# EmreAdabag/osqp

Measured on AMD Instinct MI355X. Metric: ADMM iters/sec (single QP), higher is better.
Workload: dtype f64; 1 GPU; config2 random sparse QP n=10000 m=20000 nnzA=200000 nnzPtriu=59985, one step = osqp_update_rho(0.1) + cold-started osqp_solve; adaptive_rho_interval=100, status=solved, graph_launches=4775, resident_gave_up=0, resident_slow_waits=0, parallelism=replicas x1 (a single QP does not shard)

## Files before the change

include/osqp_amd_engine.h:

```cpp
#ifndef OSQP_AMD_ENGINE_H
#define OSQP_AMD_ENGINE_H

#include "osqp_amd_types.h"

#ifdef __cplusplus
extern "C" {
#endif

#define HIPENG_OK            0
#define HIPENG_ERR_NO_DEVICE (-101)
#define HIPENG_ERR_HIP       (-102)
#define HIPENG_ERR_ARG       (-103)
#define HIPENG_ERR_ALLOC     (-104)

typedef struct hipeng hipeng;

typedef struct {
  c_float sigma;
  c_float alpha;
  c_float pcg_eps_rel;
  c_float pcg_eps_abs;
  c_int   pcg_max_iter;
  c_int   no_restart;
} hipeng_params;
// ... 14 lines not shown
} hipeng_scalars;

typedef struct {
  c_int admm_done;
  c_int pcg_iters_total;
  c_int pcg_iters_last;
  c_int pcg_iters_max;
  c_int pcg_forced;
  c_int graph_launches;
  c_int kernels_per_pcg_iter;
  c_int neg_curvature;
  c_int resident;
} hipeng_stats;

int hipeng_create(hipeng **out, const csc *P, const csc *A, const c_float *q,
                  const c_float *l, const c_float *u, const c_float *rho_vec,
                  const hipeng_params *prm, int device);
void hipeng_destroy(hipeng *e);

int hipeng_set_params(hipeng *e, const hipeng_params *prm);
int hipeng_set_scaling(hipeng *e, const c_float *D, const c_float *E, c_float c);
int hipeng_ruiz_scale(hipeng *e, c_int passes, c_float *D, c_float *E, c_float *cost,
                      c_float *q, c_float *l, c_float *u, c_float *Px, c_float *Ax);
int hipeng_matrices_changed(hipeng *e);
int hipeng_upload_q(hipeng *e, const c_float *q);
int hipeng_upload_bounds(hipeng *e, const c_float *l, const c_float *u);
int hipeng_upload_rho(hipeng *e, const c_float *rho_vec);
int hipeng_upload_matrices(hipeng *e, const csc *P, const csc *A);
int hipeng_cold_start(hipeng *e);
int hipeng_set_iterates(hipeng *e, const c_float *x, const c_float *y);
int hipeng_set_z(hipeng *e, const c_float *z);

int hipeng_run_admm(hipeng *e, c_int count);
int hipeng_residuals(hipeng *e, hipeng_scalars *out);
int hipeng_certificates(hipeng *e, c_float eps_dx, int unscaled, hipeng_scalars *inout);
int hipeng_download(hipeng *e, c_float *x, c_float *y, c_float *z, c_float *dx,
                    c_float *dy, int dy_projected);
int hipeng_get_stats(hipeng *e, hipeng_stats *st);
int hipeng_reset_stats(hipeng *e);
int hipeng_sync(hipeng *e);

int hipeng_kkt_solve(hipeng *e, c_float *b);
int hipeng_kkt_solve_unrefined(hipeng *e, c_float *b);

int hipeng_spmv(hipeng *e, int which, const c_float *x, c_float *y);
int hipeng_spmv_dev(hipeng *e, int which, const c_float *d_x, c_float *d_y);
int hipeng_time_kernel(hipeng *e, int which, int reps, double *usec);
int hipeng_kernel_bytes(hipeng *e, int which, double *bytes);
int hipeng_is_split(hipeng *e);
int hipeng_pcg_layout(hipeng *e, long long out[16]);
int hipeng_row_eliminated(hipeng *e, c_int i);
c_int hipeng_elim_count(hipeng *e);
int hipeng_resident_info(hipeng *e, long long out[16]);
int hipeng_resident_plan(const csc *P, const csc *A, int nwg, long long stats[8], int *Kptr, int *Kcol, int *kdst, long long cap,
                         unsigned short *rowpos, unsigned short *slotcol, int *wg4);
long long hipeng_resident_dump(hipeng *e, int *row, int *col, double *val, long long cap);

int hipeng_dense_invert_selftest(int n, const double *A, double *Ainv, double *ms);

typedef struct hipsens hipsens;
int hipsens_create(hipsens **out, c_int n, c_int m, c_int nnzP, c_int nnzA, int device);
void hipsens_destroy(hipsens *s);
int hipsens_set_point(hipsens *s, hipeng *pe, const c_float *x, const c_float *yact, const c_int *act,
                      const c_float *D, const c_float *E, c_float c);
int hipsens_grad(hipsens *s, hipeng *pe, const csc *P, const csc *A, const c_float *rx, const c_float *rnu,
                 c_float *dPx, c_float *dAx);
int hipsens_tan_rhs(hipsens *s, hipeng *pe, const csc *P, const csc *A, c_int ndir, const c_float *dq, const c_float *dl,
                    const c_float *du, const c_float *dPx, const c_float *dAx, c_float *g);

#ifdef __cplusplus
}
#endif
#endif
```

osqp_amd/csrc/engine.hip:

```cpp
#include <hip/hip_runtime.h>
#include <cstdio>
#include <new>
#include <cstdlib>
#include <cstring>
#include <cmath>
#include <vector>
#include <map>
#include <algorithm>
#include <mutex>
#include <condition_variable>
#include <thread>
#include <atomic>
#include <chrono>
#include "../../include/osqp_amd_engine.h"

#define TB 256
#define MAX_CHUNK 2048
#define LONG_ROW 512
#define HUGE_ROW 8192
#define MAX_PARTS 1024
#define MAX_HUGE_FOLD 4
#define INF_BOUND 1e26

#define HIPCHK(call)                                                            \
// ... 9 lines not shown
struct RowBlk { int r0, r1, k0, k1; };
#define IS_LONG(b) ((b).r1 - (b).r0 == 1 && (b).k1 - (b).k0 >= LONG_ROW)
struct __attribute__((aligned(32))) G4 { double r, w, s, m; };

struct DevMat {
  int nrows, nblk;
  int nstream;
  int nwave;
  const int    *rowptr;
  const int    *col;
  const unsigned short *col16;
  const double *val;
  const int    *split;
  const RowBlk *blk;
};

#define DENSE_MAX 128
struct DenseBlk { int c0, b, off, pitch; };
struct DenseP {
  int nblk;
  const DenseBlk *blk;
  const double *val;
};

struct State {
  int    run;
  int    done;
  int    stalled;
  int    neg_curv;
  int    iters[2];
  int    neg_curv_seen;
  int    iters_last;
  int    iters_max;
  int    iters_min;
  int    forced;
  long long iters_total;
  long long admm_done;
  double rz[2];
  double tol2;
  double gam[2], alp[2];
  int    hist_r;
  long long admm_target;
  unsigned res_epoch;
  int    res_fail;
  int    res_pipe_off;
  int    res_chk_fail;
  int    res_dbg[4];
  int    res_slow;
  int    res_slow_max;
  int    res_repub;
  int    res_slow_hist[4];
  unsigned res_slow_xcc;
  int    res_slow_last[4];
};

struct Params {
  double sigma, alpha, eps_rel, eps_abs, cinv;
  int    pcg_max_iter, use_cvec, has_scaling, pad0;
  double ex_theta;
  int    ex_h0, ex_h1;
  int    no_restart;
};

struct Ctx {
  int n, m;
  DevMat A, M;
  DevMat Mk;
  DenseP dP;
  int nh, hrow[MAX_HUGE_FOLD];
  const double *hcol;
  int gridA, gridM;
  double *xy, *z, *zt, *va, *vb, *q, *l, *u, *rho, *rhoinv, *minv, *pdiag;
  double *r, *zz, *kp, *pt0, *pt1, *dxy, *dy, *cvec;
  double *init_r, *init_z;
  double *vx, *vold;
  double *pdir, *ut;
  G4     *g4;
  int     init_stride;
  int     fin_wave_rows;
  double *vd;
  int     plain_rhs;
  const int *plain_skip;
  const unsigned short *u0map;
  double *u0pos;
  int     nelim;
  const int *erow, *ecol, *epos;
  double *rhoe, *ecoef, *edinv, *xte;
  double *D, *Dinv, *E, *Einv;
  double *part_rz, *part_rr, *part_bb, *part_pkp, *part_s0, *part_s1, *part_s2, *part_gam, *part_del;
  const double *fin_rr;
  int fin_cnt;
  double *scal;
  double *part_h;
  State  *st;
  const Params *prm;
#ifdef OSQP_AMD_TIMELINE
  unsigned long long *tl;
#endif
};

#ifdef OSQP_AMD_TIMELINE
#define TL_CAP (1 << 20)
#define TL_MARK(c, id) do { if (blockIdx.x == 0 && threadIdx.x == 0) { const unsigned long long k_ = atomicAdd((c).tl, 1ull); \
    if (k_ < TL_CAP - 2) (c).tl[1 + k_] = ((unsigned long long)(id) << 56) | (wall_clock64() & 0x00FFFFFFFFFFFFFFull); } } while (0)
#define TLK_N 10
#define TLK_DECL long long tlk_[TLK_N], tll_[2] = {0, 0}; for (int q_ = 0; q_ < TLK_N; ++q_) tlk_[q_] = 0
// ... 860 lines not shown
    TLK_AT(7, 0);
    for (int i = i0 + TB / RL; i < b.r1; i += TB / RL) {
      const double zt = row_sum_par(lprod, c.A.rowptr[i] - b.k0, c.A.rowptr[i + 1] - b.k0, rlane, RL);
      if (rlane == 0) row_update(i, zt);
    }
    __syncthreads();
  }
  for (int bi = blockIdx.x + gridDim.x; bi < c.A.nstream; bi += gridDim.x) {
    const RowBlk bb = c.A.blk[bi];
    stage_products<1>(c.A, bb, xts, nullptr, lprod, nullptr);
    __syncthreads();
    const int RLb = lanes_for(bb.r1 - bb.r0), rgb = threadIdx.x / RLb, rlb = threadIdx.x % RLb;
    for (int i = bb.r0 + rgb; i < bb.r1; i += TB / RLb) {
      const double zt = row_sum_par(lprod, c.A.rowptr[i] - bb.k0, c.A.rowptr[i + 1] - bb.k0, rlb, RLb);
      if (rlb == 0) row_update(i, zt);
    }
    __syncthreads();
  }
  if (c.fin_wave_rows) {
    const int lane = threadIdx.x & 63, wv = threadIdx.x >> 6;
    for (int bi = c.A.nstream + blockIdx.x * (TB / 64) + wv; bi < c.A.nwave; bi += gridDim.x * (TB / 64)) {
      const RowBlk lb = c.A.blk[bi];
      const double zt = wave_row_dot(c.A, lb.k0, lb.k1, [&](int cc) { return xts[cc]; });
      if (lane == 0) row_update(lb.r0, zt);
    }
  } else
  for (int bi = c.A.nstream + blockIdx.x; bi < c.A.nwave; bi += gridDim.x) {
    const RowBlk lb = c.A.blk[bi];
    const double zt = long_row_dot(c.A, lb.k0, lb.k1, xts, red);
    if (threadIdx.x == 0) row_update(lb.r0, zt);
    __syncthreads();
  }
  for (int bi = c.A.nwave + blockIdx.x; bi < c.A.nblk; bi += gridDim.x) {
    const double zt = huge_row_sum(c, bi, red);
    if (threadIdx.x == 0) row_update(c.A.blk[bi].r0, zt);
    __syncthreads();
  }
  TLK_AT(8, 0); TLK_LAST(1);
  TLK_FLUSH(c, 110, 9);
}


#define RES_TB 512
#define RES_PT (RES_TB - 64)
#define RES_MAXROWS 61
#define RES_MAXN (RES_MAXROWS * 256)
#define RES_MAXPAD 16384
#define RES_MAXLD (RES_MAXPAD / 2 / RES_TB)
#define RES_WAIT_TICKS 2000000LL
#define RES_SLOW_TICKS 5000LL
#define AUX_SC1 16
#define AUX_VOL ((int)0x80000000)
#define RES_DBG 16
#define RES_FSTRIDE 32
#define RES_GSTRIDE 16
typedef unsigned int u32x4 __attribute__((ext_vector_type(4)));
typedef unsigned int u32x2 __attribute__((ext_vector_type(2)));
struct ResWG { int r0, nr, cnt, pos; };
struct ResCtx {
  int nwg, E, npad;
  int npw;
  const unsigned short *rowpos;
  int pipe;
  int u0_direct;
  int inject;
  const ResWG *wg;
  double *val;
  const unsigned short *col;
  const unsigned char *rowl;
  const int *krp, *kcj, *kps, *kdst;
  const unsigned long long *brk;
  const unsigned short *slot0;
  const unsigned short *segrow;
  double *ubuf;
  unsigned *flags;
  int *dbg;
  double *sbuf;
};

static __device__ __forceinline__ __amdgpu_buffer_rsrc_t res_rsrc(const void *p, size_t bytes) {
  return __builtin_amdgcn_make_buffer_rsrc(const_cast<void *>(p), 0, (int)bytes, 0x00020000);
}

__device__ __forceinline__ int res_spin_check(State *st, long long &t0, int &late) {
  const long long now = wall_clock64();
  const long long el = now - t0;
  if (el < 0 || el > (1LL << 40)) { t0 = now; late = 0; return 0; }
  if (__hip_atomic_load(&st->res_fail, __ATOMIC_RELAXED, __HIP_MEMORY_SCOPE_AGENT)) return 2;
  if (el > RES_WAIT_TICKS) { if (late) return 1; late = 1; } else late = 0;
  return 0;
}
__device__ __forceinline__ void res_note(State *st, int *dbg, int g, int verdict, int kind, int nx, int first, unsigned seen, long long t0, unsigned rounds, int gidx) {
  if (verdict == 1 && atomicCAS(&st->res_dbg[0], 0, kind) == 0) { st->res_dbg[1] = nx; st->res_dbg[2] = g; st->res_dbg[3] = first; }
  int *d = dbg + (size_t)RES_DBG * g;
  const long long now = wall_clock64();
  d[3] = verdict == 1 ? kind : 3; d[4] = first; d[5] = (int)seen; d[6] = (int)(now - t0);
  d[7] = (int)__builtin_amdgcn_s_getreg((3 << 11) | 20);
  d[8] = (int)(unsigned)now; d[9] = (int)rounds; d[10] = gidx;
}
__device__ __forceinline__ void res_slow_note(State *st, long long t0, int nx, int g, int missed, int kind) {
  const long long el = wall_clock64() - t0;
  if (el > RES_SLOW_TICKS && el < (1LL << 40)) {
    atomicAdd(&st->res_slow, 1); atomicMax(&st->res_slow_max, (int)(el > 0x7fffffffLL ? 0x7fffffffLL : el));
    atomicAdd(&st->res_slow_hist[el < 20000 ? 0 : (el < 50000 ? 1 : (el < 200000 ? 2 : 3))], 1);
    atomicOr(&st->res_slow_xcc, 1u << (__builtin_amdgcn_s_getreg((3 << 11) | 20) & 15));
    st->res_slow_last[0] = nx; st->res_slow_last[1] = g; st->res_slow_last[2] = missed; st->res_slow_last[3] = kind;
  }
}

__device__ __forceinline__ int lane_int(int v, int l) { return __builtin_amdgcn_readlane(v, l); }
__global__ void __launch_bounds__(TB) k_form_K(Ctx c, ResCtx rc) {
  const double sigma = c.prm->sigma;
  if (blockIdx.x == 0 && threadIdx.x == 0) c.st->res_pipe_off = 0;
  const int lane = threadIdx.x & 63, nwaves = gridDim.x * (TB / 64);
  for (int i = blockIdx.x * (TB / 64) + (threadIdx.x >> 6); i < c.n; i += nwaves) {
    const int e0 = rc.krp[i], e1 = rc.krp[i + 1];
    const int ka = c.M.split[i], kb = c.M.rowptr[i + 1];
    for (int eb = e0; eb < e1; eb += 256) {
      int j[4]; double v[4];
#pragma unroll
      for (int q = 0; q < 4; ++q) {
        const int idx = eb + q * 64 + lane;
        j[q] = -1; v[q] = 0.0;
        if (idx < e1) {
          j[q] = rc.kcj[idx];
          const int ps = rc.kps[idx];
          v[q] = (ps >= 0 ? c.M.val[ps] : 0.0) + (j[q] == i ? sigma : 0.0);
        }
      }
      for (int kc = ka; kc < kb; kc += 64) {
        const bool on = kc + lane < kb;
        const int kk = on ? c.M.col[kc + lane] - c.n : 0;
        const double ai = on ? c.M.val[kc + lane] : 0.0, rk = on ? c.rhoe[kk] : 0.0;
        const int p0 = on ? c.A.rowptr[kk] : 0, p1 = on ? c.A.rowptr[kk + 1] : 0;
        const int cnt = min(64, kb - kc);
        for (int q = 0; q < cnt; ++q) {
          const double a_i = lane_value(ai, q), r = lane_value(rk, q);
          const int s0 = lane_int(p0, q), s1 = lane_int(p1, q);
          for (int ec = s0; ec < s1; ec += 64) {
            const bool eon = ec + lane < s1;
            const int cj = eon ? c.A.col[ec + lane] : -1;
            const double av = eon ? c.A.val[ec + lane] : 0.0;
            const int len = min(64, s1 - ec);
            for (int e = 0; e < len; ++e) {
              const int cjb = lane_int(cj, e);
              const double t = r * (a_i * lane_value(av, e));
#pragma unroll
              for (int q4 = 0; q4 < 4; ++q4) if (j[q4] == cjb) v[q4] += t;
            }
          }
        }
      }
      const bool igone = c.nelim && c.erow[i] >= 0;
#pragma unroll
      for (int q = 0; q < 4; ++q) {
        const int idx = eb + q * 64 + lane;
        if (idx < e1) {
          const bool gone = c.nelim && (igone || c.erow[j[q]] >= 0);
          rc.val[rc.kdst[idx]] = gone ? (j[q] == i ? 1.0 : 0.0) : v[q];
        }
      }
    }
  }
}

template <int E>
__global__ void __launch_bounds__(RES_TB) k_pcg_resident(Ctx c, ResCtx rc) {
  extern __shared__ __attribute__((aligned(16))) double rlds[];
  State *st = c.st;
  TL_MARK(c, 5);
  if (st->stalled || !st->run || st->res_fail) return;
  double *uv = rlds;
  double *seg = uv + rc.npad;
  double *sc = seg + RES_TB + RES_MAXROWS;
  double *sval = sc + 8;
#ifdef OSQP_AMD_TIMELINE
  long long *tls = reinterpret_cast<long long *>(sval + 768);
#define RTL(k) do { if (blockIdx.x == 0 && threadIdx.x == 0 && nx >= 1 && nx <= 64) tls[(nx - 1) * 5 + (k)] = wall_clock64(); } while (0)
  long long *wtl = tls + 5 * 64;
#define WTL(k) do { if (blockIdx.x == 0 && (threadIdx.x & 63) == 0 && (nx == 8 || nx == 1)) wtl[(nx == 1 ? 40 : 0) + (k) * 8 + (threadIdx.x >> 6)] = wall_clock64(); } while (0)
  if (blockIdx.x == 0 && threadIdx.x == 0) wtl[80] = wall_clock64();
#else
#define RTL(k) do { } while (0)
#define WTL(k) do { } while (0)
#endif
  const int g = blockIdx.x, t = threadIdx.x, lane = t & 63, wv = t >> 6;
  const int nwg = rc.nwg, npad = rc.npad;
  const ResWG w = rc.wg[g];
  const Params prm = *c.prm;
  const unsigned ep0 = st->res_epoch;
  const bool sabotage = rc.inject > 0 && g == rc.nwg - 1 && st->admm_done + 1 == rc.inject;
  bool pipe = rc.pipe && !st->res_pipe_off && !prm.no_restart;
  const bool prod = wv != 0;
  const int tt = t - 64;
  double kv[E]; unsigned short kc[E];
#pragma unroll
  for (int k = 0; k < E; ++k) { kv[k] = 0.0; kc[k] = 0; }
  unsigned long long brk = 0ull;
  int slot0 = 0;
  if (prod) {
#pragma unroll
    for (int k = 0; k < E; ++k) {
      const size_t idx = ((size_t)g * E + k) * RES_PT + tt;
      kv[k] = rc.val[idx]; kc[k] = rc.col[idx];
    }
    brk = rc.brk[(size_t)g * RES_PT + tt];
    slot0 = rc.slot0[(size_t)g * RES_PT + tt];
  }
  int sr0 = 0, sr1 = 0;
  int ppos[4];
#pragma unroll
  for (int q = 0; q < 4; ++q) { const int o = lane + 64 * q; ppos[q] = 0; if (o < rc.nwg) { const ResWG wo = rc.wg[o]; ppos[q] = wo.pos + wo.nr; } }
  double rr0 = 0.0, bb = 0.0;
  for (int i = lane; i < c.gridM; i += 64) { rr0 += c.part_rr[i]; bb += c.part_bb[i]; }
  rr0 = wave_sum(rr0); bb = wave_sum(bb);
  const double tol2 = fmax(prm.eps_rel * prm.eps_rel * bb, prm.eps_abs * prm.eps_abs);
  if (rr0 <= tol2) {
    if (g == 0 && t == 0) { st->done = 1; st->tol2 = tol2; }
    return;
  }
  const bool own = wv == 0 && lane < w.nr;
  const int j = w.r0 + lane;
  double r_ = 0, u_ = 0, w_ = 0, p_ = 0, s_ = 0, x_ = 0, mi = 0, x0_ = 0, r0_ = 0;
  double z_ = 0, q_ = 0;
  if (own) {
    r_ = c.init_r[(size_t)j * c.init_stride]; u_ = c.init_z[j]; x_ = c.vx[j]; mi = c.minv[j];
    x0_ = x_; r0_ = r_;
    sr0 = rc.segrow[(size_t)g * (RES_MAXROWS + 1) + lane]; sr1 = rc.segrow[(size_t)g * (RES_MAXROWS + 1) + lane + 1];
  }
  if (t == 0) sc[3] = 0.0;
  __syncthreads();
  int nx = 0;
  unsigned tag = ep0;
  int par = 0;

  auto vec_exchange = [&](double val, bool ride) __attribute__((always_inline)) -> bool {
    double e0 = 0.0, e1 = 0.0, e2 = 0.0;
    ++nx; tag = ep0 + (unsigned)nx; par = (int)(tag & 1u);
    if (sabotage && nx == 3) return false;
    RTL(0);
    const __amdgpu_buffer_rsrc_t rs = res_rsrc(rc.ubuf + (size_t)par * npad, (size_t)npad * 8);
    if (wv == 0) {
      if (lane < w.nr) {
        u32x2 d; d.x = (unsigned)__double2loint(val); d.y = (unsigned)__double2hiint(val);
        __builtin_amdgcn_raw_buffer_store_b64(d, rs, (w.pos + lane) * 8, 0, AUX_SC1);
      }
      if (ride) { e0 = wave_sum(own ? r_ * u_ : 0.0); e1 = wave_sum(own ? w_ * u_ : 0.0); e2 = wave_sum(own ? r_ * r_ : 0.0); }
      if (lane < 3) {
        const double v = lane == 0 ? e0 : (lane == 1 ? e1 : e2);
        u32x2 d; d.x = (unsigned)__double2loint(v); d.y = (unsigned)__double2hiint(v);
        __builtin_amdgcn_raw_buffer_store_b64(d, rs, (w.pos + w.nr + lane) * 8, 0, AUX_SC1);
      }
      asm volatile("s_waitcnt vmcnt(0)" ::: "memory");
      if (lane == 0) __hip_atomic_store(rc.flags + (size_t)g * RES_FSTRIDE, tag, __ATOMIC_RELAXED, __HIP_MEMORY_SCOPE_AGENT);
    }
    if (wv < rc.npw) {
      const int o = t;
      bool pend = o < nwg && o != g;
      int miss16 = -1;
      unsigned seen = 0, rounds = 0;
      long long t0 = wall_clock64();
      int late = 0;
      bool gave = false;
      while (true) {
        if (pend) {
          seen = __hip_atomic_load(rc.flags + (size_t)o * RES_FSTRIDE, __ATOMIC_RELAXED, __HIP_MEMORY_SCOPE_AGENT);
          pend = (int)(seen - tag) < 0;
        }
        if (!__any(pend)) break;
        if (++rounds & 15u) { __builtin_amdgcn_s_sleep(1); continue; }
        const int verdict = res_spin_check(st, t0, late);
        if (verdict) {
          const unsigned long long miss = __ballot(pend);
          const int fl = miss ? (int)__ffsll((long long)miss) - 1 : 0;
          const unsigned sv = (unsigned)__builtin_amdgcn_readlane((int)seen, fl);
          if (lane == 0) { res_note(st, rc.dbg, g, verdict, 1, nx, miss ? 64 * wv + fl : -1, sv, t0, rounds, 0); sc[3] = 1.0; }
          gave = true;
// ... 95 lines not shown
      int late = 0;
      bool gave = false;
      while (true) {
        u32x2 gv[6];
#pragma unroll
        for (int q = 0; q < 6; ++q) if (pend & (1u << q)) gv[q] = __builtin_amdgcn_raw_buffer_load_b64(rg, (o * RES_GSTRIDE + q) * 8, 0, AUX_SC1 | AUX_VOL);
#pragma unroll
        for (int q = 0; q < 6; ++q)
          if (pend & (1u << q)) { if (gv[q].y == tag) { svw[q] = gv[q].x; pend &= ~(1u << q); } else seen = gv[q].y; }
        if (!__any(pend != 0)) break;
        asm volatile("" ::: "memory");
        if (++rounds & 15u) { __builtin_amdgcn_s_sleep(1); continue; }
        const int verdict = res_spin_check(st, t0, late);
        if (verdict) {
          const unsigned long long miss = __ballot(pend != 0);
          const int fl = miss ? (int)__ffsll((long long)miss) - 1 : 0;
          const unsigned sv = (unsigned)__builtin_amdgcn_readlane((int)seen, fl);
          const int gi = __builtin_amdgcn_readlane((int)pend, fl);
          if (lane == 0) { res_note(st, rc.dbg, g, verdict, 2, nx, miss ? 64 * wv + fl : -1, sv, t0, rounds, gi); sc[3] = 1.0; }
          gave = true;
          break;
        }
        if (rounds == 16u) { const unsigned long long ms = __ballot(pend != 0); miss16 = ms ? 64 * wv + (int)__ffsll((long long)ms) - 1 : -1; }
        if ((rounds & 63u) == 0 && wv == 0) {
          if (lane < 6) {
            const double v = lane < 2 ? pg : (lane < 4 ? pd : prr);
            const unsigned half = (lane & 1) ? (unsigned)__double2hiint(v) : (unsigned)__double2loint(v);
            __hip_atomic_store(gb + (size_t)g * RES_GSTRIDE + lane, ((unsigned long long)tag << 32) | half, __ATOMIC_RELAXED, __HIP_MEMORY_SCOPE_AGENT);
          }
          if (lane == 0) atomicAdd(&st->res_repub, 1);
        }
        if ((rounds & 255u) == 0) __builtin_amdgcn_fence(__ATOMIC_ACQUIRE, "agent");
        __builtin_amdgcn_s_sleep(1);
      }
      if (rounds >= 16u && lane == 0 && !gave) res_slow_note(st, t0, nx, g, miss16, 2);
    }
    __syncthreads();
    if (wv == 0) {
      double a0 = 0.0, a1 = 0.0, a2 = 0.0;
#pragma unroll
      for (int q = 0; q < 4; ++q)
        if (lane + 64 * q < nwg) { a0 += sval[3 * (lane + 64 * q)]; a1 += sval[3 * (lane + 64 * q) + 1]; a2 += sval[3 * (lane + 64 * q) + 2]; }
      a0 = wave_sum(a0); a1 = wave_sum(a1); a2 = wave_sum(a2);
      if (lane == 0) { sc[0] = a0; sc[1] = a1; sc[2] = a2; }
    }
    __syncthreads();
    RTL(4);
    return sc[3] == 0.0;
  };

  double gam_old = 0.0, alp_old = 0.0;
  int iters = 0;
  bool conv = false, bad = false, failed = false;
  int mode = pipe ? 0 : 3;
  int check_why = 0;
  int checks3 = 0;
  bool have_u0 = rc.u0_direct;
  while (true) {
    double val = u_, m_ = 0.0;
    if (mode == 1) { m_ = mi * w_; val = m_; }
    else if (mode == 2) val = x_ - x0_;
    if (have_u0) { ++nx; tag = ep0 + (unsigned)nx; par = (int)(tag & 1u); load_u0(); have_u0 = false; }
    else if (!vec_exchange(val, mode == 1)) { failed = true; break; }
    WTL(0);
    products_issue();
    WTL(1);
    CgStep cs{};
    if (mode == 1 && wv == 0) {
      double a0 = 0.0, a1 = 0.0, a2 = 0.0;
#pragma unroll
      for (int q = 0; q < 4; ++q) if (lane + 64 * q < nwg) { a0 += uv[ppos[q]]; a1 += uv[ppos[q] + 1]; a2 += uv[ppos[q] + 2]; }
      const double gam = wave_sum(a0), del = wave_sum(a1), rr = wave_sum(a2);
      cs = cg_step(rr, gam, del, gam_old, alp_old, tol2, iters, 0, prm, false);
      gam_old = gam; alp_old = cs.alpha;
      if (lane == 0) sc[4] = cs.stop ? (cs.conv ? 1.0 : 2.0) : 0.0;
    }
    WTL(2);
    const double kx = products_finish();
    WTL(3);
    if (mode == 0) { w_ = kx; mode = 1; continue; }
    if (mode == 1) {
      const double verdict = sc[4];
      if (verdict != 0.0) { check_why = verdict == 1.0 ? 0 : 1; mode = 2; continue; }
      ++iters;
      if (own) {
        z_ = cs.first ? kx : (kx + cs.beta * z_);
        q_ = cs.first ? m_ : (m_ + cs.beta * q_);
        s_ = cs.first ? w_ : (w_ + cs.beta * s_);
        p_ = cs.first ? u_ : (u_ + cs.beta * p_);
        x_ += cs.alpha * p_;
        r_ -= cs.alpha * s_;
        u_ -= cs.alpha * q_;
        w_ -= cs.alpha * z_;
      }
      WTL(4);
      if (iters >= 64) { check_why = 2; mode = 2; }
      continue;
    }
    if (mode == 2) {
      const double rt = r0_ - kx;
      if (!scal_exchange(0.0, 0.0, own ? rt * rt : 0.0)) { failed = true; break; }
      if (sc[2] <= 2.0 * tol2) { conv = true; break; }
      if (own) { r_ = rt; u_ = mi * rt; }
      gam_old = 0.0; alp_old = 0.0;
      if (check_why == 3) ++checks3;
      if (g == 0 && t == 0) { if (check_why != 2) st->res_chk_fail += 1; if (check_why < 2) st->res_pipe_off = 1; }
      __syncthreads();
      mode = 3;
      continue;
    }
    w_ = kx;
    if (!scal_exchange(own ? r_ * u_ : 0.0, own ? w_ * u_ : 0.0, own ? r_ * r_ : 0.0)) { failed = true; break; }
    const double gam = sc[0], del = sc[1], rr = sc[2];
    cs = cg_step(rr, gam, del, gam_old, alp_old, tol2, iters, 0, prm, false);
    if (cs.stop) {
      if (cs.conv && checks3 < 2) { check_why = 3; mode = 2; continue; }
      conv = cs.conv; bad = cs.bad && !cs.conv; break;
    }
    ++iters; gam_old = gam; alp_old = cs.alpha;
    if (own) {
      p_ = cs.first ? u_ : (u_ + cs.beta * p_);
      s_ = cs.first ? w_ : (w_ + cs.beta * s_);
      x_ += cs.alpha * p_;
      r_ -= cs.alpha * s_;
      u_ = mi * r_;
    }
  }
  if (failed) {
    if (t == 0) {
      __hip_atomic_store(&st->res_fail, 1, __ATOMIC_RELAXED, __HIP_MEMORY_SCOPE_AGENT);
      int *d = rc.dbg + (size_t)RES_DBG * g;
      d[0] = nx; d[1] = mode; d[2] = iters;
      if (sabotage) { d[3] = 4; d[7] = (int)__builtin_amdgcn_s_getreg((3 << 11) | 20); d[8] = (int)(unsigned)wall_clock64(); }
    }
    return;
  }
  if (own && iters > 0) c.va[j] = x_;
#ifdef OSQP_AMD_TIMELINE
  if (g == 0 && t == 0) {
    const int cnt = (nx < 64 ? nx : 64) * 5;
    const unsigned long long k0 = atomicAdd(c.tl, (unsigned long long)cnt + 1);
    if (k0 + cnt + 1 < TL_CAP - 2) {
      for (int q = 0; q < cnt; ++q) c.tl[1 + k0 + q] = ((unsigned long long)(10 + q % 5) << 56) | ((unsigned long long)tls[q] & 0x00FFFFFFFFFFFFFFull);
      c.tl[1 + k0 + cnt] = (15ull << 56) | (wall_clock64() & 0x00FFFFFFFFFFFFFFull);
    }
    if (nx >= 8) {
      const unsigned long long k1 = atomicAdd(c.tl, 80ull);
      if (k1 + 80 < TL_CAP - 2) {
        for (int q = 0; q < 40; ++q) c.tl[1 + k1 + q] = ((unsigned long long)(20 + q) << 56) | ((unsigned long long)(wtl[q] - wtl[0]) & 0x00FFFFFFFFFFFFFFull);
        for (int q = 0; q < 40; ++q) c.tl[1 + k1 + 40 + q] = ((unsigned long long)(60 + q) << 56) | ((unsigned long long)(wtl[40 + q] - wtl[80]) & 0x00FFFFFFFFFFFFFFull);
      }
    }
  }
#endif
  if (g == 0 && t == 0) {
    st->iters[0] = iters; st->iters[1] = 0;
    st->done = conv ? 1 : 2;
    if (bad) st->neg_curv = 1;
    st->tol2 = tol2;
    st->res_epoch = ep0 + (unsigned)nx;
  }
}


struct BrCtx { int nwg; const int *blk0; double *sbuf; int *dbg; };

template <int NH>
__global__ void __launch_bounds__(RES_TB) k_pcg_blockres(Ctx c, BrCtx bc) {
  constexpr int NV = 3 + NH;
  __shared__ double ul[256];
  __shared__ double red[8 * 8];
  __shared__ double tot[8];
  __shared__ double sval[256 * NV];
  State *st = c.st;
  TL_MARK(c, 6);
  if (st->stalled || !st->run || st->res_fail) return;
  const int g = blockIdx.x, t = threadIdx.x, lane = t & 63, wv = t >> 6, nwg = bc.nwg;
#ifdef OSQP_AMD_TIMELINE
  __shared__ long long btl[6 * 64];
#define BTL(k) do { if (blockIdx.x == 0 && threadIdx.x == 0 && nx >= 1 && nx <= 64) btl[(nx - 1) * 6 + (k)] = wall_clock64(); } while (0)
#else
#define BTL(k) do { } while (0)
#endif
  const Params prm = *c.prm;
  const unsigned ep0 = st->res_epoch;
  const int rl = t >> 1, h = t & 1;
  int j = -1, cb = 0, bw = 0, c0 = 0, pitch = 0; size_t off = 0;
  {
    int base = 0;
    for (int q = bc.blk0[g]; q < bc.blk0[g + 1]; ++q) {
      const DenseBlk d = c.dP.blk[q];
      if (rl >= base && rl < base + d.b) { j = d.c0 + (rl - base); cb = base; bw = d.b; c0 = d.c0; off = (size_t)d.off; pitch = d.pitch; }
      base += d.b;
    }
  }
  const bool row = j >= 0, own = row && h == 0;
  double dadd = 0.0, hc[NH > 0 ? NH : 1], hrho[NH > 0 ? NH : 1];
#pragma unroll
  for (int q = 0; q < NH; ++q) { hc[q] = 0.0; hrho[q] = c.rho[c.hrow[q]]; }
  if (row) {
    dadd = prm.sigma;
    for (int k = c.M.split[j]; k < c.M.rowptr[j + 1]; ++k) {
      const int i = c.M.col[k] - c.n;
      bool huge = false;
#pragma unroll
      for (int q = 0; q < NH; ++q) huge |= i == c.hrow[q];
      if (!huge) { const double a = c.M.val[k]; dadd += c.rho[i] * a * a; }
    }
#pragma unroll
    for (int q = 0; q < NH; ++q) hc[q] = c.hcol[(size_t)q * c.n + j];
  }
  double kv[64];
#pragma unroll
// ... 1298 lines not shown
    std::vector<int> ord((size_t)RES_PT * E, -1);
    for (int le = 0; le < w.cnt; le++) ord[le] = le;
    if (bank_sched)
    for (int wq = 0; wq < RES_PT / 64; wq++) {
      int cntb[64][32];
      for (int k = 0; k < E; k++) for (int b = 0; b < 32; b++) cntb[k][b] = 0;
      bool freec[64];
      for (int l = 0; l < 64; l++) {
        const int t = wq * 64 + l, a = t * E;
        freec[l] = a + E <= w.cnt && rowof[a] == rowof[a + E - 1];
        if (!freec[l]) for (int k = 0; k < E && a + k < w.cnt; k++) cntb[k][rowpos[Kcol[base + a + k]] & 31]++;
      }
      for (int k = 0; k < E; k++)
        for (int l = 0; l < 64; l++) {
          if (!freec[l]) continue;
          const int a = (wq * 64 + l) * E;
          int best = k, bc = 1 << 30;
          for (int q = k; q < E; q++) { const int c = cntb[k][rowpos[Kcol[base + ord[a + q]]] & 31]; if (c < bc) { bc = c; best = q; } }
          std::swap(ord[a + k], ord[a + best]);
          cntb[k][rowpos[Kcol[base + ord[a + k]]] & 31]++;
        }
    }
    int nseg = 0, next_row = 0;
    for (int t = 0; t < RES_PT; t++) {
      slot0[(size_t)g * RES_PT + t] = (unsigned short)nseg;
      unsigned long long b = 0;
      for (int k = 0; k < E; k++) {
        if (t * E + k >= w.cnt) break;
        const int le = ord[t * E + k];
        const size_t sl = ((size_t)g * E + k) * RES_PT + t;
        col[sl] = rowpos[Kcol[base + le]]; rowl[sl] = (unsigned char)rowof[le]; kdst[base + le] = (int)sl;
        while (next_row <= rowof[le]) segrow[(size_t)g * (RES_MAXROWS + 1) + next_row++] = (unsigned short)nseg;
        const bool last = k == E - 1 || t * E + k + 1 >= w.cnt || rowof[ord[t * E + k + 1]] != rowof[le];
        if (last) { b |= 1ull << k; nseg++; }
      }
      brk[(size_t)g * RES_PT + t] = b;
    }
    for (int r = next_row; r <= RES_MAXROWS; r++) segrow[(size_t)g * (RES_MAXROWS + 1) + r] = (unsigned short)nseg;
    if (nseg > RES_TB + RES_MAXROWS) seg_over = 1;
  }
  });
  if (seg_over.load()) return 0;
  const auto tb2 = std::chrono::steady_clock::now();
  if (po) {
    po->ok = true; po->nwg = nwg; po->E = E; po->npad = npad; po->nnzK = nnzK;
    po->wg = wg; po->Kptr = Kptr; po->Kcol = Kcol; po->kdst = kdst; po->rowpos = rowpos; po->col = col; po->brk = brk;
    return 0;
  }
  ResCtx rc{};
  rc.nwg = nwg; rc.E = E; rc.npad = npad;
  rc.npw = (nwg + 63) / 64;
  rc.pipe = 1;
  if (const char *x = getenv("OSQP_AMD_RESIDENT_PIPE")) rc.pipe = atoi(x) != 0;
  rc.u0_direct = 1;
  rc.inject = 0;
  if (const char *x = getenv("OSQP_AMD_RESIDENT_INJECT")) rc.inject = atoi(x);
  if (const char *x = getenv("OSQP_AMD_RESIDENT_U0")) rc.u0_direct = atoi(x) != 0;
  unsigned short *d_rowpos = nullptr;
  ResWG *d_wg = nullptr; unsigned short *d_col = nullptr, *d_slot0 = nullptr, *d_segrow = nullptr; unsigned char *d_rowl = nullptr;
  int *d_krp = nullptr, *d_kcj = nullptr, *d_kps = nullptr, *d_kdst = nullptr; unsigned long long *d_brk = nullptr;
  if (dev_alloc(e, &d_wg, wg.size()) || dev_alloc(e, &rc.val, slots) || dev_alloc(e, &d_col, slots) || dev_alloc(e, &d_rowl, slots) ||
      dev_alloc(e, &d_krp, Kptr.size()) || dev_alloc(e, &d_kcj, Kcol.size()) || dev_alloc(e, &d_kps, Kps.size()) || dev_alloc(e, &d_kdst, kdst.size()) ||
      dev_alloc(e, &d_brk, brk.size()) || dev_alloc(e, &d_slot0, slot0.size()) ||
      dev_alloc(e, &d_segrow, segrow.size()) || dev_alloc(e, &d_rowpos, rowpos.size()) || dev_alloc(e, &rc.ubuf, (size_t)2 * rc.npad) ||
      dev_alloc_polled(e, &rc.flags, (size_t)nwg * RES_FSTRIDE) || dev_alloc(e, &rc.dbg, (size_t)nwg * RES_DBG) || dev_alloc_polled(e, &rc.sbuf, (size_t)2 * nwg * RES_GSTRIDE)) return HIPENG_ERR_HIP;
#define UP(dst, src) HIPCHK(hipMemcpyAsync(dst, (src).data(), (src).size() * sizeof((src)[0]), hipMemcpyHostToDevice, e->stream))
  UP(d_wg, wg); UP(d_rowpos, rowpos); UP(d_col, col); UP(d_rowl, rowl); UP(d_krp, Kptr); UP(d_kcj, Kcol); UP(d_kps, Kps); UP(d_kdst, kdst); UP(d_brk, brk); UP(d_slot0, slot0); UP(d_segrow, segrow);
#undef UP
  HIPCHK(hipStreamSynchronize(e->stream));
  {
    double *d_u0pos = nullptr;
    if (dev_alloc(e, &d_u0pos, (size_t)rc.npad)) return HIPENG_ERR_HIP;
    e->c.u0map = d_rowpos; e->c.u0pos = d_u0pos;
  }
  rc.wg = d_wg; rc.rowpos = d_rowpos; rc.col = d_col; rc.rowl = d_rowl; rc.krp = d_krp; rc.kcj = d_kcj; rc.kps = d_kps; rc.kdst = d_kdst; rc.brk = d_brk; rc.slot0 = d_slot0; rc.segrow = d_segrow;
  e->rc = rc;
  e->res_lds = ((size_t)rc.npad + RES_TB + RES_MAXROWS + 3 + 16 + 768 + 5 * 64 + 96) * sizeof(double);
  int rcode = 0;
  switch (E) {
    case 8: rcode = res_set_lds<8>(e->res_lds); break;   case 16: rcode = res_set_lds<16>(e->res_lds); break;
    case 20: rcode = res_set_lds<20>(e->res_lds); break; case 24: rcode = res_set_lds<24>(e->res_lds); break;
    case 32: rcode = res_set_lds<32>(e->res_lds); break; case 48: rcode = res_set_lds<48>(e->res_lds); break;
    default: rcode = res_set_lds<64>(e->res_lds); break;
  }
  if (rcode) RES_NO("the launch's LDS request was refused");
  e->res_nnz = nnzK;
  e->res_on = e->res_use = true;
  if (e->trace) {
    const auto tb3 = std::chrono::steady_clock::now();
    auto ms = [](std::chrono::steady_clock::time_point a, std::chrono::steady_clock::time_point b) { return std::chrono::duration<double, std::milli>(b - a).count(); };
    fprintf(stderr, "[osqp_amd] resident PCG: nnz(K)=%lld, %d workgroups x %d threads x %d entries, %zu B LDS; host: pattern %.0f ms, layout %.0f ms, upload %.0f ms\n",
            nnzK, nwg, RES_TB, E, e->res_lds, ms(tb0, tb1), ms(tb1, tb2), ms(tb2, tb3));
  }
  return 0;
}


static bool blocks_eligible(hipeng *e) {
  if (e->dP_blks.empty()) return false;
  int next = 0;
  for (const DenseBlk &d : e->dP_blks) { if (d.c0 != next || d.b > DENSE_MAX) return false; next += d.b; }
  if (next != e->n) return false;
  if ((int)e->A.blk.size() - e->A.nwave != (int)e->hrows.size()) return false;
  std::vector<char> ishuge(std::max(1, e->m), 0);
  for (int hr : e->hrows) ishuge[hr] = 1;
  for (int i = 0; i < e->m; i++) if (!ishuge[i] && e->A.rowptr[i + 1] - e->A.rowptr[i] != 1) return false;
// ... 1062 lines not shown
  for (const ResWG &w : po.wg) { if (w.nr) stats[4]++; stats[5] = std::max<long long>(stats[5], w.nr); stats[6] = std::max<long long>(stats[6], w.cnt); }
  if (Kptr) std::copy(po.Kptr.begin(), po.Kptr.end(), Kptr);
  if (po.nnzK <= cap) { if (Kcol) std::copy(po.Kcol.begin(), po.Kcol.end(), Kcol); if (kdst) std::copy(po.kdst.begin(), po.kdst.end(), kdst); }
  else if (Kcol || kdst) return HIPENG_ERR_ARG;
  if (rowpos) std::copy(po.rowpos.begin(), po.rowpos.end(), rowpos);
  if (slotcol) std::copy(po.col.begin(), po.col.end(), slotcol);
  if (wg4) for (size_t g = 0; g < po.wg.size(); g++) { wg4[4 * g] = po.wg[g].r0; wg4[4 * g + 1] = po.wg[g].nr; wg4[4 * g + 2] = po.wg[g].cnt; wg4[4 * g + 3] = po.wg[g].pos; }
  return 0;
}

#ifdef OSQP_AMD_TIMELINE
extern "C" long long hipeng_timeline(hipeng *e, unsigned long long *out, long long cap) {
  if (!e || !out) return -1;
  if (hipSetDevice(e->device) != hipSuccess || hipStreamSynchronize(e->stream) != hipSuccess) return -1;
  unsigned long long cnt = 0;
  if (hipMemcpy(&cnt, e->c.tl, sizeof cnt, hipMemcpyDeviceToHost) != hipSuccess) return -1;
  const long long k = (long long)std::min<unsigned long long>(std::min<unsigned long long>(cnt, TL_CAP - 2), (unsigned long long)cap);
  if (k > 0 && hipMemcpy(out, e->c.tl + 1, (size_t)k * sizeof(unsigned long long), hipMemcpyDeviceToHost) != hipSuccess) return -1;
  if (hipMemset(e->c.tl, 0, sizeof(unsigned long long)) != hipSuccess) return -1;
  return k;
}
#endif

extern "C" int hipeng_is_split(hipeng *e) { return e && e->split ? 1 : 0; }
extern "C" int hipeng_pcg_layout(hipeng *e, long long out[16]) {
  if (!e || !out) return HIPENG_ERR_ARG;
  for (int k = 0; k < 16; k++) out[k] = 0;
  const HostMat &B = (!e->dP_blks.empty() || !e->hrows.empty()) ? e->Mr : e->M;
  out[0] = (long long)e->dP_blks.size();
  for (const DenseBlk &d : e->dP_blks) out[1] += d.b;
  out[2] = e->A.nstream; out[3] = e->A.nwave - e->A.nstream; out[4] = (long long)e->A.blk.size() - e->A.nwave;
  out[5] = (long long)e->hrows.size(); out[6] = e->split ? 1 : 0;
  out[7] = e->A.d_col16 != nullptr; out[8] = e->M.d_col16 != nullptr; out[9] = B.d_col16 != nullptr;
  out[10] = B.nwave - B.nstream; out[11] = e->c.gridA; out[12] = e->c.gridM;
  return 0;
}
extern "C" int hipeng_row_eliminated(hipeng *e, c_int i) { return e && !e->ecol.empty() && i >= 0 && i < (c_int)e->ecol.size() && e->ecol[(size_t)i] >= 0 ? 1 : 0; }
extern "C" c_int hipeng_elim_count(hipeng *e) { return e ? e->c.nelim : 0; }

extern "C" int hipeng_resident_info(hipeng *e, long long out[16]) {
  if (!e || !out) return HIPENG_ERR_ARG;
  HIPCHK(hipSetDevice(e->device));
  State s;
  if (read_state(e, &s)) return HIPENG_ERR_HIP;
  out[0] = e->res_on; out[1] = e->res_on && e->res_fails < 3; out[2] = e->rc.E; out[3] = e->rc.nwg; out[4] = e->res_nnz; out[5] = (long long)e->res_lds;
  out[6] = std::max(s.iters[0], s.iters[1]); out[7] = s.res_pipe_off; out[8] = s.res_chk_fail; out[9] = e->res_kind; out[10] = e->res_gave_up; out[11] = e->res_slow + s.res_slow;
  out[12] = std::max<long long>(e->res_slow_max, s.res_slow_max); out[13] = e->res_repub + s.res_repub; out[14] = e->res_fails; out[15] = e->res_kind == 3 ? e->bd.kc : 0;
  if (e->res_kind == 2) { out[2] = 64; out[3] = e->bc.nwg; out[4] = 0; out[5] = 0; }
  if (e->res_kind == 3) { out[2] = 0; out[3] = e->c.dP.nblk; out[4] = 0; out[5] = 0; }
  if (e->res_kind == 4) { out[2] = 0; out[3] = e->dd.na; out[4] = (long long)e->dd.nap * e->dd.nap; out[5] = e->dd_chol ? 1 : 0; out[15] = e->dd.nb2; }
  return 0;
}

extern "C" long long hipeng_resident_dump(hipeng *e, int *row, int *col, double *val, long long cap) {
  if (!e || e->res_kind != 1 || !row || !col || !val) return HIPENG_ERR_ARG;
  if (hipSetDevice(e->device) != hipSuccess || hipStreamSynchronize(e->stream) != hipSuccess) return HIPENG_ERR_HIP;
  const ResCtx &rc = e->rc;
  const size_t slots = (size_t)rc.nwg * rc.E * RES_PT;
  const long long nnz = e->res_nnz;
  if (nnz > cap) return HIPENG_ERR_ARG;
  std::vector<double> v(slots); std::vector<int> krp(e->n + 1), kcj((size_t)nnz), kdst((size_t)nnz);
  if (hipMemcpy(v.data(), rc.val, slots * sizeof(double), hipMemcpyDeviceToHost) != hipSuccess ||
      hipMemcpy(krp.data(), rc.krp, krp.size() * sizeof(int), hipMemcpyDeviceToHost) != hipSuccess ||
      hipMemcpy(kcj.data(), rc.kcj, kcj.size() * sizeof(int), hipMemcpyDeviceToHost) != hipSuccess ||
      hipMemcpy(kdst.data(), rc.kdst, kdst.size() * sizeof(int), hipMemcpyDeviceToHost) != hipSuccess) return HIPENG_ERR_HIP;
  long long k = 0;
  for (int i = 0; i < e->n; i++)
    for (int q = krp[i]; q < krp[i + 1]; q++) { row[k] = i; col[k] = kcj[q]; val[k] = v[kdst[q]]; k++; }
  return k;
}

extern "C" int hipeng_kernel_bytes(hipeng *e, int which, double *bytes) {
  if (!e || !bytes) return HIPENG_ERR_ARG;
  const double n = e->n, m = e->m;
  const double nnzA = (double)e->A.val.size();
  const double nnzPtriu = (double)e->P_toM_up.size();
  if (which == 0)      *bytes = nnzA * 12 + (m + 1) * 4 + 8 * (12 * n + 2 * m);
  else if (which == 1) *bytes = (nnzA + nnzPtriu) * 12 + (n + 1) * 4 + 8 * ((n + m) + 2 * n);
  else                 *bytes = 0;
  return 0;
}

#include "kkt_sens.h"
#include "rowpart_native.h"
```

Before: 7966 ADMM iters/s.

## Speculatively overlap PCG convergence check with next iteration in resident kernel

Measured after the change: 8077 ADMM iters/s (median of 6 runs). 1.4% higher.

```diff
diff --git a/include/osqp_amd_engine.h b/include/osqp_amd_engine.h
--- a/include/osqp_amd_engine.h
+++ b/include/osqp_amd_engine.h
@@ -90,6 +90,7 @@
 int hipeng_row_eliminated(hipeng *e, c_int i);
 c_int hipeng_elim_count(hipeng *e);
 int hipeng_resident_info(hipeng *e, long long out[16]);
+int hipeng_resident_trips(hipeng *e, long long out[8]);
 int hipeng_resident_plan(const csc *P, const csc *A, int nwg, long long stats[8], int *Kptr, int *Kcol, int *kdst, long long cap,
                          unsigned short *rowpos, unsigned short *slotcol, int *wg4);
 long long hipeng_resident_dump(hipeng *e, int *row, int *col, double *val, long long cap);
diff --git a/osqp_amd/csrc/engine.hip b/osqp_amd/csrc/engine.hip
--- a/osqp_amd/csrc/engine.hip
+++ b/osqp_amd/csrc/engine.hip
@@ -85,6 +85,9 @@
   int    res_slow_hist[4];
   unsigned res_slow_xcc;
   int    res_slow_last[4];
+  long long res_trips, res_solves, res_pred_hit, res_pred_miss;
+  int    res_pred_win[3];
+  int    res_pred_off;
 };
 
 struct Params {
@@ -1051,6 +1054,7 @@
 #define AUX_SC1 16
 #define AUX_VOL ((int)0x80000000)
 #define RES_DBG 16
+#define RES_PRED_WINDOW 16
 #define RES_FSTRIDE 32
 #define RES_GSTRIDE 16
 typedef unsigned int u32x4 __attribute__((ext_vector_type(4)));
@@ -1061,6 +1065,8 @@
   int npw;
   const unsigned short *rowpos;
   int pipe;
+  int predict;
+  double pred_margin;
   int u0_direct;
   int inject;
   const ResWG *wg;
@@ -1110,7 +1116,10 @@
 __device__ __forceinline__ int lane_int(int v, int l) { return __builtin_amdgcn_readlane(v, l); }
 __global__ void __launch_bounds__(TB) k_form_K(Ctx c, ResCtx rc) {
   const double sigma = c.prm->sigma;
-  if (blockIdx.x == 0 && threadIdx.x == 0) c.st->res_pipe_off = 0;
+  if (blockIdx.x == 0 && threadIdx.x == 0) {
+    c.st->res_pipe_off = 0;
+    c.st->res_pred_off = 0; c.st->res_pred_win[0] = 0; c.st->res_pred_win[1] = 0; c.st->res_pred_win[2] = 0;
+  }
   const int lane = threadIdx.x & 63, nwaves = gridDim.x * (TB / 64);
   for (int i = blockIdx.x * (TB / 64) + (threadIdx.x >> 6); i < c.n; i += nwaves) {
     const int e0 = rc.krp[i], e1 = rc.krp[i + 1];
@@ -1190,6 +1199,7 @@
   const unsigned ep0 = st->res_epoch;
   const bool sabotage = rc.inject > 0 && g == rc.nwg - 1 && st->admm_done + 1 == rc.inject;
   bool pipe = rc.pipe && !st->res_pipe_off && !prm.no_restart;
+  bool predict = pipe && rc.predict && !st->res_pred_off;
   const bool prod = wv != 0;
   const int tt = t - 64;
   double kv[E]; unsigned short kc[E];
@@ -1220,8 +1230,12 @@
   }
   const bool own = wv == 0 && lane < w.nr;
   const int j = w.r0 + lane;
-  double r_ = 0, u_ = 0, w_ = 0, p_ = 0, s_ = 0, x_ = 0, mi = 0, x0_ = 0, r0_ = 0;
-  double z_ = 0, q_ = 0;
+  double rs_rest[11] = {0, 0, 0, 0, 0, 0, 0, 0, 0, 0, 0};
+#define RES_ROWSTATE(i) (*((i) < E ? &kv[(i) < E ? (i) : 0] : &rs_rest[i]))
+  double &r_ = RES_ROWSTATE(0), &u_ = RES_ROWSTATE(1), &w_ = RES_ROWSTATE(2), &p_ = RES_ROWSTATE(3), &s_ = RES_ROWSTATE(4), &x_ = RES_ROWSTATE(5);
+  double &mi = RES_ROWSTATE(6), &x0_ = RES_ROWSTATE(7), &r0_ = RES_ROWSTATE(8);
+  double &z_ = RES_ROWSTATE(9), &q_ = RES_ROWSTATE(10);
+#undef RES_ROWSTATE
   if (own) {
     r_ = c.init_r[(size_t)j * c.init_stride]; u_ = c.init_z[j]; x_ = c.vx[j]; mi = c.minv[j];
     x0_ = x_; r0_ = r_;
@@ -1423,13 +1437,16 @@
   double gam_old = 0.0, alp_old = 0.0;
   int iters = 0;
   bool conv = false, bad = false, failed = false;
+  double rr_prev = 0.0;
+  bool pred = false;
+  int pred_hit = 0, pred_miss = 0;
   int mode = pipe ? 0 : 3;
   int check_why = 0;
   int checks3 = 0;
   bool have_u0 = rc.u0_direct;
   while (true) {
     double val = u_, m_ = 0.0;
-    if (mode == 1) { m_ = mi * w_; val = m_; }
+    if (mode == 1) { m_ = mi * w_; val = pred ? x_ - x0_ : m_; }
     else if (mode == 2) val = x_ - x0_;
     if (have_u0) { ++nx; tag = ep0 + (unsigned)nx; par = (int)(tag & 1u); load_u0(); have_u0 = false; }
     else if (!vec_exchange(val, mode == 1)) { failed = true; break; }
@@ -1443,16 +1460,28 @@
       for (int q = 0; q < 4; ++q) if (lane + 64 * q < nwg) { a0 += uv[ppos[q]]; a1 += uv[ppos[q] + 1]; a2 += uv[ppos[q] + 2]; }
       const double gam = wave_sum(a0), del = wave_sum(a1), rr = wave_sum(a2);
       cs = cg_step(rr, gam, del, gam_old, alp_old, tol2, iters, 0, prm, false);
-      gam_old = gam; alp_old = cs.alpha;
-      if (lane == 0) sc[4] = cs.stop ? (cs.conv ? 1.0 : 2.0) : 0.0;
+      if (lane == 0) sc[4] = (cs.stop ? (cs.conv ? 1.0 : 2.0) : 0.0) + (pred ? 4.0 : 0.0);
+      if (pred) { pred = false; predict = false; }
+      else {
+        gam_old = gam; alp_old = cs.alpha;
+        pred = predict && !cs.stop && iters >= 1 && rr * rr <= rc.pred_margin * tol2 * rr_prev;
+        rr_prev = rr;
+      }
     }
     WTL(2);
     const double kx = products_finish();
     WTL(3);
-    if (mode == 0) { w_ = kx; mode = 1; continue; }
+    if (mode == 0) { if (!prod) w_ = kx; mode = 1; continue; }
     if (mode == 1) {
-      const double verdict = sc[4];
-      if (verdict != 0.0) { check_why = verdict == 1.0 ? 0 : 1; mode = 2; continue; }
+      const int verdict = (int)sc[4];
+      if (verdict == 4) { ++pred_miss; continue; }
+      if (verdict != 0) {
+        check_why = (verdict & 3) == 1 ? 0 : 1; mode = 2;
+        if (verdict < 4) continue;
+        ++pred_hit;
+      }
+    }
+    if (mode == 1) {
       ++iters;
       if (own) {
         z_ = cs.first ? kx : (kx + cs.beta * z_);
@@ -1465,7 +1494,7 @@
         w_ -= cs.alpha * z_;
       }
       WTL(4);
-      if (iters >= 64) { check_why = 2; mode = 2; }
+      if (iters >= 64) { check_why = 2; mode = 2; pred = false; }
       continue;
     }
     if (mode == 2) {
@@ -1480,7 +1509,7 @@
       mode = 3;
       continue;
     }
-    w_ = kx;
+    if (!prod) w_ = kx;
     if (!scal_exchange(own ? r_ * u_ : 0.0, own ? w_ * u_ : 0.0, own ? r_ * r_ : 0.0)) { failed = true; break; }
     const double gam = sc[0], del = sc[1], rr = sc[2];
     cs = cg_step(rr, gam, del, gam_old, alp_old, tol2, iters, 0, prm, false);
@@ -1530,6 +1559,13 @@
     if (bad) st->neg_curv = 1;
     st->tol2 = tol2;
     st->res_epoch = ep0 + (unsigned)nx;
+    st->res_trips += nx; st->res_solves += 1; st->res_pred_hit += pred_hit; st->res_pred_miss += pred_miss;
+    if (rc.predict && !st->res_pred_off) {
+      const int ws = st->res_pred_win[0] + 1, wh = st->res_pred_win[1] + pred_hit, wm = st->res_pred_win[2] + pred_miss;
+      const bool full = ws >= RES_PRED_WINDOW;
+      if (full && wm > wh) st->res_pred_off = 1;
+      st->res_pred_win[0] = full ? 0 : ws; st->res_pred_win[1] = full ? 0 : wh; st->res_pred_win[2] = full ? 0 : wm;
+    }
   }
 }
 
@@ -2934,6 +2970,9 @@
   rc.npw = (nwg + 63) / 64;
   rc.pipe = 1;
   if (const char *x = getenv("OSQP_AMD_RESIDENT_PIPE")) rc.pipe = atoi(x) != 0;
+  rc.predict = 1; rc.pred_margin = 1.0;
+  if (const char *x = getenv("OSQP_AMD_RESIDENT_PREDICT")) rc.predict = atoi(x) != 0;
+  if (const char *x = getenv("OSQP_AMD_RESIDENT_PREDICT_MARGIN")) { const double v = atof(x); if (v > 0.0) rc.pred_margin = v; }
   rc.u0_direct = 1;
   rc.inject = 0;
   if (const char *x = getenv("OSQP_AMD_RESIDENT_INJECT")) rc.inject = atoi(x);
@@ -4102,6 +4141,16 @@
   return 0;
 }
 
+extern "C" int hipeng_resident_trips(hipeng *e, long long out[8]) {
+  if (!e || !out) return HIPENG_ERR_ARG;
+  HIPCHK(hipSetDevice(e->device));
+  State s;
+  if (read_state(e, &s)) return HIPENG_ERR_HIP;
+  out[0] = s.res_trips; out[1] = s.res_solves; out[2] = s.res_pred_hit; out[3] = s.res_pred_miss;
+  out[4] = s.res_pred_off; out[5] = e->res_kind == 1 ? e->rc.predict : 0; out[6] = s.res_pred_win[0]; out[7] = s.res_pred_win[2] - s.res_pred_win[1];
+  return 0;
+}
+
 extern "C" long long hipeng_resident_dump(hipeng *e, int *row, int *col, double *val, long long cap) {
   if (!e || e->res_kind != 1 || !row || !col || !val) return HIPENG_ERR_ARG;
   if (hipSetDevice(e->device) != hipSuccess || hipStreamSynchronize(e->stream) != hipSuccess) return HIPENG_ERR_HIP;
```
